# marvinli00/genie2

Hardware: AMD Instinct MI355X
Metric: denoise-steps/sec (N=256, T=1000, batch=8) (higher is better)
Workload: dtype f32 (pair-stack products as 3 f16 MFMAs on 2xf16-split operands, f32 accumulate); 1 GPU; unconditional N=256, T=1000, batch=8 per GPU, random-init base Denoiser (15.7M params), scale=0.6, reverse-loop steps 995..676; parallelism=replica per GPU x1, no data-path collective

## Files before the change

genie2_amd/csrc/common.h:

```cpp
#pragma once
#include <hip/hip_runtime.h>
#include <stdint.h>
#include "../../include/genie_hip.h"

typedef float f32x16 __attribute__((ext_vector_type(16)));
typedef float f32x4 __attribute__((ext_vector_type(4)));

#define GENIE_LN_EPS 1e-5f

#ifdef __HIPCC__

__device__ __forceinline__ f32x16 mfma_8k(const float4 a, const float4 b, f32x16 c) {
    c = __builtin_amdgcn_mfma_f32_32x32x2f32(a.x, b.x, c, 0, 0, 0);
    c = __builtin_amdgcn_mfma_f32_32x32x2f32(a.y, b.y, c, 0, 0, 0);
    c = __builtin_amdgcn_mfma_f32_32x32x2f32(a.z, b.z, c, 0, 0, 0);
    c = __builtin_amdgcn_mfma_f32_32x32x2f32(a.w, b.w, c, 0, 0, 0);
    return c;
}

__device__ __forceinline__ f32x16 zero16() {
    f32x16 z;
#pragma unroll
    for (int i = 0; i < 16; ++i) z[i] = 0.f;
    return z;
// ... 188 lines not shown
    int32_t *f_aatype, *f_rmask, *f_ridx, *f_cidx;
    float *f_pos;
    uint8_t *f_fsm, *f_fstm, *f_ifm;
    float *rmaskf;

    void* ws; size_t ws_bytes;
    float *p, *acm, *bcm, *xcm, *pstatic, *ipa_bias;
    float *spart;
    unsigned *pmax;
    float *xsingle, *s0, *s, *s1, *s2, *h1, *h2, *pij, *proj, *cat;
    float *kT, *v, *qp, *kpT, *vp;
    float *vf, *vmax;
    float *ta_tb, *ta_xn, *ta_qkvg;
    float *rots_w, *trans_w;
    int32_t* tsteps;
    float *loop_z;

    bool prof;
    struct ProfRec { int cls; hipEvent_t a, b; };
    ProfRec* prof_recs; int prof_n, prof_cap;
    double prof_ms[KC_COUNT]; int64_t prof_cnt[KC_COUNT];
    double train_gemm_flop;

    hipStream_t st2; hipEvent_t ev_fork, ev_join;
};

void launch_single_input(genie_ctx* h, hipStream_t st, const int32_t* timesteps);
void launch_gemm_rows(genie_ctx* h, hipStream_t st, const float* A, int lda, int M, int K,
                      const float* Wp, int Nout, const float* bias, const float* res, int ldr,
                      const float* rowmask, int relu, float* out, int ldo, int prof_class = KC_GEMM_ROWS);
// ... 4 lines not shown
                      const int8_t* codes);
void launch_trimul(genie_ctx* h, hipStream_t st, const TriMulW& w, bool outgoing);
void launch_pair_transition(genie_ctx* h, hipStream_t st, const PairLayerW& w);
void launch_triatt(genie_ctx* h, hipStream_t st, const TriAttW& w, bool starting);
void triatt_ws_floats(const genie_dims_t& d, int B, int N, size_t* tb, size_t* xn, size_t* qkvg);
bool launch_pair_stack_fused(genie_ctx* h, hipStream_t st, float* tap_trimul_out0, float* tap_layer0);
void launch_ipa_bias(genie_ctx* h, hipStream_t st);
void launch_ipa_prep(genie_ctx* h, hipStream_t st, int b0 = 0, int nb = -1);
void launch_ipa_attn(genie_ctx* h, hipStream_t st, int layer, const float* head_w, int b0 = 0, int nb = -1);
size_t ipa_vf_floats(const genie_dims_t& d, int B, int N);
bool ipa_attn_splits(const genie_ctx* h);
void launch_q_sample(genie_ctx* h, hipStream_t st, const float* x0, const float* z, const float* c0, const float* c1, float* trans_out);
void launch_training_loss(genie_ctx* h, hipStream_t st, const float* zp, const float* z, float w, float* losses, float* grad);
void launch_adam(hipStream_t st, size_t n, float* p, const float* g, float* m, float* v, double lr, double b1, double b2, double eps, int step);
void launch_any_nonzero(genie_ctx* h, hipStream_t st, const uint8_t* x, size_t n, unsigned* flag);
bool launch_struct_tail(genie_ctx* h, hipStream_t st, const StructLayerW& S, const float* trans_in, float* z_out, int b0 = 0, int nb = -1);
bool struct_tail_fused(const genie_ctx* h, const StructLayerW& S);
void launch_bb_update(genie_ctx* h, hipStream_t st, const StructLayerW& w, const float* trans_in,
                      float* z_out);
void launch_frenet(genie_ctx* h, hipStream_t st, int mode, int step, float scale, float* trans,
                   float* rots, const float* z, const float* eps);
void launch_fill_i32(genie_ctx* h, hipStream_t st, int32_t* p, int n, int v);
void train_ws_free(genie_ctx* h);

void prof_begin(genie_ctx* h, hipStream_t st, int cls);
void prof_end(genie_ctx* h, hipStream_t st);

struct ProfScope {
    genie_ctx* h; hipStream_t st; bool on;
    ProfScope(genie_ctx* h_, hipStream_t st_, int cls, bool enable = true) : h(h_), st(st_), on(enable && h_->prof) { if (on) prof_begin(h, st, cls); }
    ~ProfScope() { if (on) prof_end(h, st); }
};
```

genie2_amd/csrc/genie_api.hip:

```cpp
#include <stdio.h>
#include <stdlib.h>
#include <string.h>
#include <math.h>
#include <algorithm>
#include <cmath>
#include <new>
#include <string>
#include <vector>

#include "common.h"

void pair_kernels_init();
void pair_fused_kernels_init();
void single_kernels_init(const genie_dims_t& d, int n_max);
void launch_scale_copy(genie_ctx* h, hipStream_t st, const float* in, float* out, int n, float s);
size_t ipa_attn_lds(const genie_dims_t& d, int N);

static char g_create_err[512] = "";

#define SET_ERR(h, ...) do { snprintf((h)->err, sizeof((h)->err), __VA_ARGS__); } while (0)
#define HIP_TRY(h, call) do { hipError_t e_ = (call); if (e_ != hipSuccess) { \
    SET_ERR(h, "%s failed: %s (%s:%d)", #call, hipGetErrorString(e_), __FILE__, __LINE__); return GENIE_E_HIP; } } while (0)

static const char* kKernelNames[KC_COUNT] = {
// ... 96 lines not shown
}

static void free_batch(genie_ctx* h) {
    if (h->ws) { (void)hipFree(h->ws); h->ws = nullptr; h->ws_bytes = 0; }
    h->have_feats = false;
}

void genie_destroy(genie_handle_t h) {
    if (!h) return;
    (void)hipSetDevice(h->device);
    free_batch(h);
    train_ws_free(h);
    if (h->wdev) (void)hipFree(h->wdev);
    if (h->hxdev) (void)hipFree(h->hxdev);
    if (h->pos_tab) (void)hipFree(h->pos_tab);
    free(h->sched_host);
    for (int i = 0; i < h->prof_n; ++i) { (void)hipEventDestroy(h->prof_recs[i].a); (void)hipEventDestroy(h->prof_recs[i].b); }
    free(h->prof_recs);
    if (h->st2) { (void)hipStreamSynchronize(h->st2); (void)hipEventDestroy(h->ev_fork); (void)hipEventDestroy(h->ev_join); (void)hipStreamDestroy(h->st2); }
    delete[] h->pair;
    delete[] h->st;
    delete h;
}

const char* genie_last_error(genie_handle_t h) { return h ? h->err : g_create_err; }
size_t genie_workspace_bytes(genie_handle_t h) { return h ? h->ws_bytes : 0; }

namespace {
struct Img {
    std::vector<float> data;
// ... 380 lines not shown
    HIP_TRY(h, hipMemcpy(h->sched, sched, s * sizeof(float), hipMemcpyHostToDevice));
    free(h->sched_host);
    h->sched_host = (float*)malloc(s * sizeof(float));
    memcpy(h->sched_host, sched, s * sizeof(float));
    h->n_pos = n_pos;
    h->n_chain = n_chain;
    h->have_tables = true;
    return GENIE_OK;
}

__global__ void k_mask_to_float(const int32_t* m, float* f, int n) {
    const int i = blockIdx.x * blockDim.x + threadIdx.x;
    if (i < n) f[i] = (float)m[i];
}

int genie_prepare_features(genie_handle_t h, genie_stream_t stream, int B, int N, const genie_features_t* f) {
    if (!h || !f || B < 1 || N < 2) return GENIE_E_ARG;
    if (!h->have_weights) { SET_ERR(h, "genie_prepare_features: weights not loaded"); return GENIE_E_STATE; }
    const genie_dims_t& d = h->d;
    if (ipa_attn_lds(d, N) > 160 * 1024) { SET_ERR(h, "N = %d exceeds the attention kernel's LDS budget", N); return GENIE_E_ARG; }
    if ((size_t)24 * N * sizeof(float) > 160 * 1024) { SET_ERR(h, "N = %d exceeds the Frenet kernel's LDS budget (96 B per residue)", N); return GENIE_E_ARG; }
    {
        const size_t np = (size_t)((N + 31) / 32 * 32);
        const size_t pair_bytes = (size_t)B * np * np * d.c_p * sizeof(float);
        if (pair_bytes >= ((size_t)1 << 31)) {
            SET_ERR(h, "batch %d x N %d: a pair tensor of %zu bytes exceeds the 2 GiB the kernels address; split the batch", B, N, pair_bytes);
            return GENIE_E_ARG;
        }
    }
    HIP_TRY(h, hipSetDevice(h->device));
// ... 25 lines not shown
        size_t ntb, nxn, nq;
        triatt_ws_floats(d, B, N, &ntb, &nxn, &nq);
        want(&h->ta_tb, ntb * 4); want(&h->ta_xn, nxn * 4); want(&h->ta_qkvg, nq * 4);
    }
    size_t total = 0;
    for (auto& s : segs) total += s.bytes;
    if (total > h->ws_bytes) {
        free_batch(h);
        hipError_t e = hipMalloc(&h->ws, total);
        if (e != hipSuccess) { SET_ERR(h, "workspace hipMalloc(%zu MB) failed: %s", total >> 20, hipGetErrorString(e)); return GENIE_E_NOMEM; }
        h->ws_bytes = total;
    }
    size_t off = 0;
    for (auto& s : segs) { *s.p = (char*)h->ws + off; off += s.bytes; }
    h->B = B; h->N = N; h->NP = NP;

    HIP_TRY(h, hipMemcpyAsync(h->f_aatype, f->aatype, M * 20 * 4, hipMemcpyDeviceToDevice, st));
    HIP_TRY(h, hipMemcpyAsync(h->f_pos, f->atom_positions, M * 3 * 4, hipMemcpyDeviceToDevice, st));
    HIP_TRY(h, hipMemcpyAsync(h->f_rmask, f->residue_mask, M * 4, hipMemcpyDeviceToDevice, st));
    HIP_TRY(h, hipMemcpyAsync(h->f_ridx, f->residue_index, M * 4, hipMemcpyDeviceToDevice, st));
    HIP_TRY(h, hipMemcpyAsync(h->f_cidx, f->chain_index, M * 4, hipMemcpyDeviceToDevice, st));
    HIP_TRY(h, hipMemcpyAsync(h->f_fsm, f->fixed_sequence_mask, M, hipMemcpyDeviceToDevice, st));
    HIP_TRY(h, hipMemcpyAsync(h->f_fstm, f->fixed_structure_mask, P, hipMemcpyDeviceToDevice, st));
    HIP_TRY(h, hipMemcpyAsync(h->f_ifm, f->interface_mask, M, hipMemcpyDeviceToDevice, st));
    hipLaunchKernelGGL(k_mask_to_float, dim3((unsigned)((M + 255) / 256)), dim3(256), 0, st, h->f_rmask, h->rmaskf, (int)M);
    HIP_TRY(h, hipMemsetAsync(h->acm, 0, (size_t)B * cp * NP * NP * 4, st));
    HIP_TRY(h, hipMemsetAsync(h->vf, 0, ipa_vf_floats(d, B, N) * 4, st));
    HIP_TRY(h, hipMemsetAsync(h->bcm, 0, (size_t)B * cp * NP * NP * 4, st));
    single_kernels_init(d, N);
    {
        unsigned any = 0;
        HIP_TRY(h, hipMemsetAsync(h->pmax, 0, sizeof(unsigned), st));
        launch_any_nonzero(h, st, h->f_fstm, P, h->pmax);
        HIP_TRY(h, hipMemcpyAsync(&any, h->pmax, sizeof(unsigned), hipMemcpyDeviceToHost, st));
        HIP_TRY(h, hipStreamSynchronize(st));
        h->has_motif = any != 0;
    }
    launch_pair_static(h, st);
    HIP_TRY(h, hipGetLastError());
    h->have_feats = true;
    return GENIE_OK;
}

static int denoise_internal(genie_ctx* h, hipStream_t st, const float* trans, const float* rots, const int32_t* ts_dev,
                            const int8_t* codes, float* z_out, const genie_taps_t* taps) {
    const genie_dims_t& d = h->d;
    const int B = h->B, N = h->N, M = B * N;
    const size_t P = (size_t)M * N;
    const int cs = d.c_s, cp = d.c_p;
    const int ldx = (single_in(d) + 7) / 8 * 8;
    auto d2d = [&](void* dst, const void* src, size_t bytes) { return hipMemcpyAsync(dst, src, bytes, hipMemcpyDeviceToDevice, st); };

    h->hx_launches = 1;
    launch_scale_copy(h, st, trans, h->trans_w, M * 3, d.rescale);
    HIP_TRY(h, d2d(h->rots_w, rots, (size_t)M * 9 * 4));

    launch_single_input(h, st, ts_dev);
    launch_gemm_rows(h, st, h->xsingle, ldx, M, ldx, h->single_w, cs, nullptr, nullptr, 0, h->rmaskf, 0, h->s0, cs);
    if (taps && taps->s) HIP_TRY(h, d2d(taps->s, h->s0, (size_t)M * cs * 4));

    launch_gemm_rows(h, st, h->s0, cs, M, cs, h->pij_w, 2 * cp, nullptr, nullptr, 0, nullptr, 0, h->pij, 2 * cp);
    launch_pair_init(h, st, h->trans_w, h->rots_w, codes);
    if (taps && taps->p_init) HIP_TRY(h, d2d(taps->p_init, h->p, P * cp * 4));

    const bool fused = launch_pair_stack_fused(h, st, taps ? taps->p_trimul_out0 : nullptr, taps ? taps->p_layer0 : nullptr);
    for (int l = 0; l < (fused ? 0 : d.n_pair_transform_layer); ++l) {
        launch_trimul(h, st, h->pair[l].out, true);
        if (l == 0 && taps && taps->p_trimul_out0) HIP_TRY(h, d2d(taps->p_trimul_out0, h->p, P * cp * 4));
        launch_trimul(h, st, h->pair[l].in, false);
        if (d.n_head_tri > 0) {
            launch_triatt(h, st, h->pair[l].ta_start, true);
            launch_triatt(h, st, h->pair[l].ta_end, false);
            if (l == 0 && taps && taps->p_tri_att0) HIP_TRY(h, d2d(taps->p_tri_att0, h->p, P * cp * 4));
        }
        launch_pair_transition(h, st, h->pair[l]);
        if (l == 0 && taps && taps->p_layer0) HIP_TRY(h, d2d(taps->p_layer0, h->p, P * cp * 4));
    }
    if (taps && taps->p) HIP_TRY(h, d2d(taps->p, h->p, P * cp * 4));

    launch_ipa_bias(h, st);
    HIP_TRY(h, d2d(h->s, h->s0, (size_t)M * cs * 4));
    if (taps && taps->states) HIP_TRY(h, d2d(taps->states, h->s0, (size_t)M * cs * 4));
    int n_state = 1;
    const int nproj = ipa_proj_n(d), ncat = ipa_cat_n(d);
    bool split = h->st2 && B >= 2 && M >= 1024 && ipa_attn_splits(h) && !getenv("GENIE_NO_STRUCT_SPLIT");
    for (int l = 0; split && l < d.n_structure_layer; ++l) split = struct_tail_fused(h, h->st[l]);
    const int n_half = split ? 2 : 1;
    const int n_layers = d.n_structure_block * d.n_structure_layer;
    hipStream_t hstream[2] = {st, h->st2};
    if (split) {
        HIP_TRY(h, hipEventRecord(h->ev_fork, st));
        HIP_TRY(h, hipStreamWaitEvent(h->st2, h->ev_fork, 0));
    }
    for (int half = 0; half < n_half; ++half) {
        hipStream_t hs = hstream[half];
        const int b0 = (int)((long long)B * half / n_half), nb = (int)((long long)B * (half + 1) / n_half) - b0;
        const size_t r0 = (size_t)b0 * N, nr = (size_t)nb * N;
        int li = 0;
        for (int blk = 0; blk < d.n_structure_block; ++blk) {
            for (int l = 0; l < d.n_structure_layer; ++l, ++li) {
                const StructLayerW& S = h->st[l];
                const bool last = li == n_layers - 1;
                launch_gemm_rows(h, hs, h->s + r0 * cs, cs, (int)nr, cs, S.proj_w, nproj, S.proj_b, nullptr, 0, nullptr, 0, h->proj + r0 * nproj, nproj);
                launch_ipa_prep(h, hs, b0, nb);
                launch_ipa_attn(h, hs, l, S.head_w, b0, nb);
                if (li == 0 && taps && taps->ipa_cat0) HIP_TRY(h, hipMemcpyAsync(taps->ipa_cat0 + r0 * ncat, h->cat + r0 * ncat, nr * ncat * 4, hipMemcpyDeviceToDevice, hs));
                auto state_tap = [&]() -> hipError_t {
                    return (taps && taps->states) ? hipMemcpyAsync(taps->states + (size_t)(1 + li) * M * cs + r0 * cs, h->s + r0 * cs, nr * cs * 4, hipMemcpyDeviceToDevice, hs)
                                                  : hipSuccess;
                };
                if (launch_struct_tail(h, hs, S, last ? trans : nullptr, last ? z_out : nullptr, b0, nb)) { HIP_TRY(h, state_tap()); continue; }
                launch_gemm_rows(h, hs, h->cat, ncat, M, ncat, S.out_w, cs, S.out_b, h->s, cs, nullptr, 0, h->s1, cs);
                launch_layernorm_rows(h, hs, h->s1, h->s2, M, cs, S.ln_ipa_g, S.ln_ipa_b);
                launch_gemm_rows(h, hs, h->s2, cs, M, cs, S.t1_w, cs, S.t1_b, nullptr, 0, nullptr, 1, h->h1, cs);
                launch_gemm_rows(h, hs, h->h1, cs, M, cs, S.t2_w, cs, S.t2_b, nullptr, 0, nullptr, 1, h->h2, cs);
                launch_gemm_rows(h, hs, h->h2, cs, M, cs, S.t3_w, cs, S.t3_b, h->s2, cs, nullptr, 0, h->s1, cs);
                launch_layernorm_rows(h, hs, h->s1, h->s, M, cs, S.ln_tr_g, S.ln_tr_b);
                launch_bb_update(h, hs, S, last ? trans : nullptr, last ? z_out : nullptr);
                HIP_TRY(h, state_tap());
            }
        }
    }
    if (split) {
        for (int q = 1; q < n_half; ++q) {
            HIP_TRY(h, hipEventRecord(h->ev_join, hstream[q]));
            HIP_TRY(h, hipStreamWaitEvent(st, h->ev_join, 0));
// ... 75 lines not shown
                      int first_step, int last_step, float* trans_io, float* rots_io, float* record) {
    if (int rc = check_ready(h, "genie_sample_loop")) return rc;
    const int T = h->d.n_timestep;
    if (!noise || !trans_io || !rots_io || first_step > T || last_step < 1 || first_step < last_step) {
        SET_ERR(h, "genie_sample_loop: bad argument");
        return GENIE_E_ARG;
    }
    hipStream_t st = (hipStream_t)stream;
    const size_t n3 = (size_t)h->B * h->N * 3, nn = (size_t)h->B * h->N * h->N;
    if (first_step == T) {
        HIP_TRY(h, hipMemcpyAsync(trans_io, noise, n3 * 4, hipMemcpyDeviceToDevice, st));
        launch_frenet(h, st, 0, 0, 0.f, trans_io, rots_io, nullptr, nullptr);
    }
    int it = 0;
    for (int step = first_step; step >= last_step; --step, ++it) {
        launch_fill_i32(h, st, h->tsteps, h->B, step);
        const int8_t* codes = quat_codes ? quat_codes + (size_t)it * nn : nullptr;
        if (int rc = denoise_internal(h, st, trans_io, rots_io, h->tsteps, codes, h->loop_z, nullptr)) return rc;
        const float* eps = (step == 1) ? nullptr : noise + (size_t)(T - step + 1) * n3;
        launch_frenet(h, st, 1, step, scale, trans_io, rots_io, h->loop_z, eps);
        if (record) HIP_TRY(h, hipMemcpyAsync(record + (size_t)it * n3, trans_io, n3 * 4, hipMemcpyDeviceToDevice, st));
    }
    HIP_TRY(h, hipGetLastError());
    return GENIE_OK;
}

int genie_set_math(genie_handle_t h, int mode) {
    if (!h || (mode != GENIE_MATH_F32 && mode != GENIE_MATH_HX)) return GENIE_E_ARG;
    h->hx = mode == GENIE_MATH_HX;
    return GENIE_OK;
}
int genie_get_math(genie_handle_t h) { return h && h->hx ? GENIE_MATH_HX : GENIE_MATH_F32; }

int genie_profile_enable(genie_handle_t h, int enable) {
    if (!h) return GENIE_E_ARG;
// ... 27 lines not shown
```

genie2_amd/csrc/pair_hx_kernels.hip:

```cpp
#include "hx_pair.h"


template <int NW>
__global__ __launch_bounds__(NW * 64, NW == 8 ? 1 : 2) void k_pair_transition_hx(
    float* __restrict__ z, const float* __restrict__ rmask, const unsigned char* __restrict__ wimg,
    const float* __restrict__ b1s, const float* __restrict__ b2s, int N, long long M, int n_hb, float sx, float c1, float c2, int rev) {
    extern __shared__ __attribute__((aligned(16))) unsigned char smb[];
    float* sb1 = reinterpret_cast<float*>(smb + 2 * HX_STAGE_BYTES);
    const int lane = threadIdx.x & 63, wave = UNI(threadIdx.x >> 6);
    const int h = lane >> 5, pl = lane & 31;
    const int n_wt = (int)((M + 31) / 32);
    const int n_tiles = (n_wt + NW - 1) / NW;
    const rsrc_t rw = hx_rsrc(wimg, (unsigned)(n_hb * HX_STAGE_BYTES));
    const rsrc_t rz = hx_rsrc(z, (unsigned)(M * 512));
    const rsrc_t rnull = hx_rsrc(z, 0u);
    const int lane16 = lane * 16;
    constexpr int PW = 32 / NW;
    auto issue = [&](int hb, int buf) {
#pragma unroll
        for (int q = 0; q < PW; ++q) {
            const int p = PW * wave + q;
            hx_dma(rw, smb + buf * HX_STAGE_BYTES + p * 1024, lane16, hb * HX_STAGE_BYTES + p * 1024);
        }
    };
// ... 807 lines not shown
    }
#pragma unroll
    for (int o = 32; o > 0; o >>= 1) amax = fmaxf(amax, __shfl_xor(amax, o));
    if (lane == 0 && __float_as_uint(amax) > *reinterpret_cast<volatile unsigned*>(pmax)) atomicMax(pmax, __float_as_uint(amax));
}

bool launch_ipa_bias_hx(genie_ctx* h, hipStream_t st) {
    const int LH = h->d.n_structure_layer * h->d.n_head_ipa;
    if (!h->hx || LH > 96) return false;
    const HxGemmW* w = nullptr;
    for (int i = 0; i < h->n_hxg; ++i)
        if (h->hxg[i].w == h->ipa_bias_w) w = &h->hxg[i];
    if (!w) return false;
    const int N = h->N, n_tiles = h->B * N * ((N + 31) / 32);
    const int grid = n_tiles / 4 < 2 * hx_num_cu() ? (n_tiles + 3) / 4 : 2 * hx_num_cu();
    (void)hipMemsetAsync(h->pmax, 0, sizeof(unsigned), st);
    hipLaunchKernelGGL(k_ipa_bias_hx, dim3(grid), dim3(256), IB_UNITS * 2048 + 96 * 4, st, h->p, w->img, w->inv_s, h->ipa_bias_b, h->ipa_bias,
                       h->B, N, LH, n_tiles, (int)(h->hx_launches & 1), h->pmax);
    return true;
}

void pair_hx_kernels_init() {
#define HX_ATTR(k) (void)hipFuncSetAttribute(reinterpret_cast<const void*>(k), hipFuncAttributeMaxDynamicSharedMemorySize, HX_LDS_BYTES)
    HX_ATTR((k_trimul_proj_hx<true, 8>)); HX_ATTR((k_trimul_proj_hx<false, 8>));
    HX_ATTR(k_trimul_out_hx_r<8>);
    (void)hipFuncSetAttribute(reinterpret_cast<const void*>(k_trimul_contract_hx_big), hipFuncAttributeMaxDynamicSharedMemorySize, 4 * CB_PLANE);
#undef HX_ATTR
    (void)hipFuncSetAttribute(reinterpret_cast<const void*>(k_pair_transition_hx<8>), hipFuncAttributeMaxDynamicSharedMemorySize, HX_LDS_BYTES);
    (void)hipFuncSetAttribute(reinterpret_cast<const void*>(k_ipa_bias_hx), hipFuncAttributeMaxDynamicSharedMemorySize, IB_UNITS * 2048 + 96 * 4);
}
```

genie2_amd/csrc/pair_kernels.hip:

```cpp
#include "common.h"

#define LDZ 132


template <bool AMAX = false>
__device__ __forceinline__ float load_tile64(float* tile, const float* __restrict__ src, size_t row_stride,
                                             int nvalid, int tid) {
    const int c4 = tid & 31;
    const int r0 = tid >> 5;
    float4 v[8];
    const int last = max(nvalid - 1, 0);
#pragma unroll
    for (int u = 0; u < 8; ++u) {
        const int r = min(r0 + 8 * u, last);
        v[u] = *reinterpret_cast<const float4*>(src + (size_t)r * row_stride + c4 * 4);
    }
#pragma unroll
    for (int u = 0; u < 8; ++u) {
        const int r = r0 + 8 * u;
        if (r >= nvalid) v[u] = make_float4(0.f, 0.f, 0.f, 0.f);
        *reinterpret_cast<float4*>(tile + r * LDZ + c4 * 4) = v[u];
    }
    float am = 0.f;
    if constexpr (AMAX) {
// ... 181 lines not shown
#pragma unroll
    for (int q = 0; q < 10; ++q) {
        const int k = part + 4 * q;
        if (k < nbin) frow[k] = (x[q] / s) * pm;
    }
}

#define LDF 52
template <bool TABLE>
__global__ __launch_bounds__(256) void k_pair_init(const float* __restrict__ trans, const float* __restrict__ rots,
                                                   const int8_t* __restrict__ codes, const float* __restrict__ rmask,
                                                   const uint8_t* __restrict__ fstm, const float* __restrict__ pij,
                                                   const float* __restrict__ pstatic, const float* __restrict__ wt,
                                                   float* __restrict__ p, int N, float dmin, float dstep, int nbin,
                                                   const int32_t* __restrict__ ridx, const int32_t* __restrict__ cidx,
                                                   const float* __restrict__ relpos_t, int relpos_k) {
    __shared__ __attribute__((aligned(16))) float ft[64 * LDF];
    __shared__ float pmk[64];
    __shared__ int dsel[64];
    __shared__ float same[64];
    const int tid = threadIdx.x, lane = tid & 63, wave = tid >> 6;
    const int ntile = (N + 63) >> 6;
    const int st = blockIdx.x % ntile;
    const int i = (blockIdx.x / ntile) % N;
    const int b = blockIdx.x / (ntile * N);
    const int t0 = st * 64;
    const int nvalid = min(64, N - t0);
    {
        const int jl = tid >> 2, part = tid & 3;
        float* frow = ft + jl * LDF;
        if (jl < nvalid) {
            const int j = t0 + jl;
            const float pm = rmask[b * N + i] * rmask[b * N + j];
            const float* xi = trans + ((size_t)b * N + i) * 3;
            const float* xj = trans + ((size_t)b * N + j) * 3;
            const float dx = xi[0] - xj[0], dy = xi[1] - xj[1], dz = xi[2] - xj[2];
            const float d = sqrtf(1e-10f + ((dx * dx + dy * dy) + dz * dz));
            soft_bins(frow, d, dmin, dstep, nbin, pm, part);
            if (part == 0) {
                const float* Ri = rots + ((size_t)b * N + i) * 9;
                const float* Rj = rots + ((size_t)b * N + j) * 9;
                float r[9];
// ... 139 lines not shown
        hipLaunchKernelGGL(k_pair_static<true>, grid, dim3(256), 0, st, h->f_pos, h->f_ridx, h->f_cidx, h->f_fsm, h->f_fstm,
                           h->relpos_t, h->motif_w, h->pstatic, N, h->d.relpos_k, h->d.template_dist_min,
                           h->d.template_dist_step, h->d.template_dist_n_bin);
    else
        hipLaunchKernelGGL(k_pair_static<false>, grid, dim3(256), 0, st, h->f_pos, h->f_ridx, h->f_cidx, h->f_fsm, h->f_fstm,
                           h->relpos_t, h->motif_w, h->pstatic, N, h->d.relpos_k, h->d.template_dist_min,
                           h->d.template_dist_step, h->d.template_dist_n_bin);
}

void launch_pair_init(genie_ctx* h, hipStream_t st, const float* trans, const float* rots, const int8_t* codes) {
    ProfScope ps(h, st, KC_PAIR_INIT);
    const int N = h->N, ntile = (N + 63) / 64;
    if (!h->has_motif)
        hipLaunchKernelGGL(k_pair_init<true>, dim3(h->B * N * ntile), dim3(256), 0, st, trans, rots, codes, h->rmaskf, h->f_fstm,
                           h->pij, h->pstatic, h->templ_w, h->p, N, h->d.template_dist_min, h->d.template_dist_step,
                           h->d.template_dist_n_bin, h->f_ridx, h->f_cidx, h->relpos_t, h->d.relpos_k);
    else
        hipLaunchKernelGGL(k_pair_init<false>, dim3(h->B * N * ntile), dim3(256), 0, st, trans, rots, codes, h->rmaskf, h->f_fstm,
                           h->pij, h->pstatic, h->templ_w, h->p, N, h->d.template_dist_min, h->d.template_dist_step,
                           h->d.template_dist_n_bin, h->f_ridx, h->f_cidx, h->relpos_t, h->d.relpos_k);
}

void launch_trimul_proj_wl(genie_ctx* h, hipStream_t st, const TriMulW& w, bool outgoing);
void launch_trimul_out_wl(genie_ctx* h, hipStream_t st, const TriMulW& w);
void launch_pair_transition_wl(genie_ctx* h, hipStream_t st, const PairLayerW& w);

void launch_trimul_hx(genie_ctx* h, hipStream_t st, const TriMulW& w, bool outgoing);
void launch_trimul(genie_ctx* h, hipStream_t st, const TriMulW& w, bool outgoing) {
    if (h->hx) { launch_trimul_hx(h, st, w, outgoing); return; }
    const int NP = h->NP;
    {
        ProfScope ps(h, st, KC_TRIMUL_PROJ);
        launch_trimul_proj_wl(h, st, w, outgoing);
    }
    {
// ... 24 lines not shown

void launch_pair_transition_hx(genie_ctx* h, hipStream_t st, const PairLayerW& w);
void launch_pair_transition(genie_ctx* h, hipStream_t st, const PairLayerW& w) {
    ProfScope ps(h, st, KC_PAIR_TRANSITION);
    if (h->hx) launch_pair_transition_hx(h, st, w);
    else launch_pair_transition_wl(h, st, w);
}

bool launch_ipa_bias_hx(genie_ctx* h, hipStream_t st);
void launch_ipa_bias(genie_ctx* h, hipStream_t st) {
    ProfScope ps(h, st, KC_IPA_BIAS);
    if (launch_ipa_bias_hx(h, st)) return;
    const int N = h->N, ntile = (N + 127) / 128;
    const int LH = h->d.n_structure_layer * h->d.n_head_ipa;
    const size_t lds = 128 * LDZ * sizeof(float);
    (void)hipMemsetAsync(h->pmax, 0, sizeof(unsigned), st);
    hipLaunchKernelGGL(k_ipa_bias, dim3(h->B * N * ntile), dim3(256), lds, st, h->p, h->ipa_bias_w, h->ipa_bias_b, h->ipa_bias,
                       h->B, N, LH, h->hx ? (int)(h->hx_launches & 1) : 0, h->pmax);
}

void pair_wl_kernels_init();
void pair_hx_kernels_init();
void pair_kernels_init() {
    pair_wl_kernels_init();
    pair_hx_kernels_init();
    (void)hipFuncSetAttribute(reinterpret_cast<const void*>(k_trimul_contract<2>), hipFuncAttributeMaxDynamicSharedMemorySize,
                        2 * 2 * 128 * LDK * sizeof(float));
    (void)hipFuncSetAttribute(reinterpret_cast<const void*>(k_ipa_bias), hipFuncAttributeMaxDynamicSharedMemorySize,
                        128 * LDZ * sizeof(float));
}
```

genie2_amd/csrc/single_kernels.hip:

```cpp
#include <algorithm>
#include <type_traits>
#include "hx.h"

__global__ void k_single_input(float* __restrict__ x, int ldx, const float* __restrict__ pos_tab, int n_pos, int c_pos,
                               const float* __restrict__ chain_tab, int n_chain, int c_chain,
                               const float* __restrict__ t_tab, int c_t, const int32_t* __restrict__ timesteps,
                               const int32_t* __restrict__ ridx, const int32_t* __restrict__ cidx,
                               const int32_t* __restrict__ aatype, const uint8_t* __restrict__ fsm,
                               const uint8_t* __restrict__ ifm, int N, int n_timestep) {
    const int row = blockIdx.x;
    const int b = row / N;
    float* xr = x + (size_t)row * ldx;
    const int ri = min(max(ridx[row], 0), n_pos - 1);
    const int ci = min(max(cidx[row], 0), n_chain - 1);
    const int ts = min(max(timesteps[b], 0), n_timestep);
    const float f = fsm[row] ? 1.f : 0.f;
    const int o1 = c_pos, o2 = o1 + c_chain, o3 = o2 + c_t, o4 = o3 + 20;
    for (int c = threadIdx.x; c < ldx; c += blockDim.x) {
        float v;
        if (c < o1) v = pos_tab[(size_t)ri * c_pos + c];
        else if (c < o2) v = chain_tab[(size_t)ci * c_chain + (c - o1)];
        else if (c < o3) v = t_tab[(size_t)ts * c_t + (c - o2)];
        else if (c < o4) v = (float)aatype[(size_t)row * 20 + (c - o3)] * f;
        else if (c < o4 + 2) v = f;
// ... 961 lines not shown
            for (int k = 0; k < 9; ++k) R[k] = Rn[k];
            t[0] = tx; t[1] = ty; t[2] = tz;
            if (z_out) {
                z_out[(size_t)row * 3 + 0] = trans_in[(size_t)row * 3 + 0] - tx * inv_rescale;
                z_out[(size_t)row * 3 + 1] = trans_in[(size_t)row * 3 + 1] - ty * inv_rescale;
                z_out[(size_t)row * 3 + 2] = trans_in[(size_t)row * 3 + 2] - tz * inv_rescale;
            }
        }
    }
}

__global__ __launch_bounds__(256) void k_p_sample_frenet(int mode, float* __restrict__ trans, float* __restrict__ rots,
                                                         const float* __restrict__ z, const float* __restrict__ eps,
                                                         const int32_t* __restrict__ rmask, const int32_t* __restrict__ cidx,
                                                         int N, float alpha, float sqrt_alpha, float somac, float sqrt_beta,
                                                         float scale) {
    extern __shared__ __attribute__((aligned(16))) float sm[];
    float* x = sm;
    float* tv = x + 3 * N;
    float* base = tv + 3 * N;
    float* st1 = base + 9 * N;
    __shared__ int s_len;
    const int b = blockIdx.x, tid = threadIdx.x;
    float* tr = trans + (size_t)b * N * 3;
    if (tid == 0) s_len = 0;
    __syncthreads();
    int cnt = 0;
    for (int n = tid; n < N; n += 256) cnt += rmask[b * N + n];
    atomicAdd(&s_len, cnt);
    if (mode == 1) {
        const float w_z = (1.0f - alpha) / somac;
        const float inv_sa = 1.0f / sqrt_alpha;
        for (int u = tid; u < 3 * N; u += 256) {
            const float m = (float)rmask[b * N + u / 3];
            float v = inv_sa * (tr[u] - w_z * z[(size_t)b * N * 3 + u]);
            v = v * m;
            if (eps) { v = v + scale * sqrt_beta * eps[(size_t)b * N * 3 + u]; v = v * m; }
            x[u] = v;
            tr[u] = v;
        }
    } else {
        for (int u = tid; u < 3 * N; u += 256) x[u] = tr[u];
    }
    __syncthreads();
    const int len = s_len;
    for (int n = tid; n < N - 1; n += 256) {
        const float dx = x[3 * n + 3] - x[3 * n], dy = x[3 * n + 4] - x[3 * n + 1], dz = x[3 * n + 5] - x[3 * n + 2];
        const float nr = sqrtf(1e-10f + ((dx * dx + dy * dy) + dz * dz));
        tv[3 * n] = dx / nr; tv[3 * n + 1] = dy / nr; tv[3 * n + 2] = dz / nr;
    }
    __syncthreads();
    for (int n = tid; n < N; n += 256) {
        float R[9] = {1.f, 0.f, 0.f, 0.f, 1.f, 0.f, 0.f, 0.f, 1.f};
        if (n >= 1 && n < len - 1) {
            const int m = n - 1;
            const float ax = tv[3 * m], ay = tv[3 * m + 1], az = tv[3 * m + 2];
            const float bx = tv[3 * m + 3], by = tv[3 * m + 4], bz = tv[3 * m + 5];
            float cx = ay * bz - az * by, cy = az * bx - ax * bz, cz = ax * by - ay * bx;
// ... 13 lines not shown
        int srcn = n;
        if (n < len && (n == 0 || ch[n] != ch[n - 1])) srcn = n + 1;
#pragma unroll
        for (int k = 0; k < 9; ++k) st1[9 * n + k] = (srcn < N) ? base[9 * srcn + k] : ((k % 4 == 0) ? 1.f : 0.f);
    }
    __syncthreads();
    float* ro = rots + (size_t)b * N * 9;
    for (int n = tid; n < N; n += 256) {
        int k = n;
        if (n < len) {
            while (k >= 0 && (k == len - 1 || ch[k] != ch[k + 1])) --k;
            if (k < 0) k = N - 1;
        }
#pragma unroll
        for (int q = 0; q < 9; ++q) ro[9 * n + q] = st1[9 * k + q];
    }
}

__global__ void k_fill_i32(int32_t* p, int n, int v) {
    const int i = blockIdx.x * blockDim.x + threadIdx.x;
    if (i < n) p[i] = v;
}

__global__ void k_scale_copy(const float* __restrict__ in, float* __restrict__ out, int n, float s) {
    const int i = blockIdx.x * blockDim.x + threadIdx.x;
    if (i < n) out[i] = in[i] * s;
}

template <int H, int C, int PQ, int PV, int Q, int MF>
__global__ __launch_bounds__(MF ? 128 * Q : 512, MF ? 4 : 1) void k_ipa_attn_q(const float* __restrict__ proj, int ldp, const float* __restrict__ kT,
                                                    const float* __restrict__ v, const float* __restrict__ qp,
                                                    const float* __restrict__ kpT, const float* __restrict__ vp,
                                                    const float* __restrict__ bias, const float* __restrict__ z,
                                                    const float* __restrict__ rots, const float* __restrict__ trans,
                                                    const float* __restrict__ rmask, const float* __restrict__ head_w,
                                                    float* __restrict__ cat, int B, int N, int layer, int rev,
// ... 550 lines not shown
    const int M = h->B * h->N;
    hipLaunchKernelGGL(k_bb_update, dim3((M + 3) / 4), dim3(256), 0, st, h->s, h->d.c_s, w.bb_w, w.bb_b, h->rots_w, h->trans_w,
                       M, trans_in, z_out, 1.0f / h->d.rescale);
}

static size_t struct_rows_lds() { return (size_t)2 * 32 * SR_LD * 4 + 6 * (2 * 32 * GH_ROWB + 32 * 4) + 32 * 12 * 4; }
static const HxGemmW* hx_image(const genie_ctx* h, const float* Wp) {
    for (int i = 0; i < h->n_hxg; ++i)
        if (h->hxg[i].w == Wp) return &h->hxg[i];
    return nullptr;
}
bool struct_tail_fused(const genie_ctx* h, const StructLayerW& S) {
    if (!h->hx || h->d.c_s != 384 || getenv("GENIE_NO_STRUCT_FUSE")) return false;
    return hx_image(h, S.out_w) && hx_image(h, S.t1_w) && hx_image(h, S.t2_w) && hx_image(h, S.t3_w);
}
bool launch_struct_tail(genie_ctx* h, hipStream_t st, const StructLayerW& S, const float* trans_in, float* z_out, int b0, int nb) {
    if (!struct_tail_fused(h, S)) return false;
    const HxGemmW *w0 = hx_image(h, S.out_w), *w1 = hx_image(h, S.t1_w), *w2 = hx_image(h, S.t2_w), *w3 = hx_image(h, S.t3_w);
    if (nb < 0) { b0 = 0; nb = h->B; }
    const int Mall = h->B * h->N, M = nb * h->N, cs = h->d.c_s, ncat = h->d.n_head_ipa * (h->d.c_p + h->d.c_hidden_ipa + 4 * h->d.n_v_point);
    const size_t zs = (size_t)Mall * cs, r0 = (size_t)b0 * h->N;
    {
        ProfScope ps(h, st, KC_GEMM_ROWS);
        hipLaunchKernelGGL(k_gemm_rows_hx, dim3((M + 31) / 32, (cs + 127) / 128, SR_KSPLIT), dim3(256), 0, st, h->cat + r0 * ncat, ncat, M, ncat,
                           w0->img, cs, w0->inv_s, nullptr, nullptr, 0, nullptr, 0, h->spart + r0 * cs, cs, zs);
    }
    ProfScope ps(h, st, KC_STRUCT_ROWS);
    const int nrb = (M + 31) / 32;
    hipLaunchKernelGGL((k_struct_rows_hx<12>), dim3(nrb + 64), dim3(768), struct_rows_lds(), st, h->spart + r0 * cs, SR_KSPLIT, zs, S.out_b, h->s + r0 * cs,
                       S.ln_ipa_g, S.ln_ipa_b, w1->img, w1->inv_s, S.t1_b, w2->img, w2->inv_s, S.t2_b, w3->img, w3->inv_s, S.t3_b,
                       S.ln_tr_g, S.ln_tr_b, S.bb_w, S.bb_b, h->s + r0 * cs, h->rots_w + r0 * 9, h->trans_w + r0 * 3, M, trans_in ? trans_in + r0 * 3 : nullptr,
                       z_out ? z_out + r0 * 3 : nullptr, 1.0f / h->d.rescale, nrb);
    return true;
}

void launch_q_sample(genie_ctx* h, hipStream_t st, const float* x0, const float* z, const float* c0, const float* c1, float* trans_out) {
    ProfScope ps(h, st, KC_MISC);
    const int total = h->B * h->N * 3;
    hipLaunchKernelGGL(k_q_sample, dim3((total + 255) / 256), dim3(256), 0, st, x0, z, c0, c1, trans_out, h->N * 3, total);
}
void launch_training_loss(genie_ctx* h, hipStream_t st, const float* zp, const float* z, float w, float* losses, float* grad) {
    ProfScope ps(h, st, KC_MISC);
    float* stats = h->loop_z;
    hipLaunchKernelGGL(k_training_loss, dim3(h->B), dim3(256), 0, st, zp, z, h->f_rmask, h->f_fsm, h->B, h->N, w, losses, stats, grad);
    hipLaunchKernelGGL(k_training_loss_mean, dim3(1), dim3(64), 0, st, stats, h->B, losses);
}

void launch_frenet(genie_ctx* h, hipStream_t st, int mode, int step, float scale, float* trans, float* rots, const float* z,
                   const float* eps) {
    ProfScope ps(h, st, KC_P_SAMPLE);
    float al = 1.f, sa = 1.f, so = 1.f, sb = 0.f;
    if (mode == 1) {
        const int T1 = h->d.n_timestep + 1;
        al = h->sched_host[0 * T1 + step];
        sa = h->sched_host[1 * T1 + step];
        so = h->sched_host[2 * T1 + step];
        sb = h->sched_host[3 * T1 + step];
    }
    const size_t lds = (size_t)(3 + 3 + 9 + 9) * h->N * sizeof(float);
    hipLaunchKernelGGL(k_p_sample_frenet, dim3(h->B), dim3(256), lds, st, mode, trans, rots, z, eps, h->f_rmask, h->f_cidx, h->N,
                       al, sa, so, sb, scale);
}

int genie_frenet_frames(genie_stream_t stream, int B, int N, const float* coords, const int32_t* chains, const int32_t* mask,
                        float* rots_out) {
    if (!coords || !chains || !mask || !rots_out || B < 1 || N < 2) return GENIE_E_ARG;
    const size_t lds = (size_t)24 * N * sizeof(float);
    if (lds > 160 * 1024) return GENIE_E_ARG;
    if (lds > 64 * 1024)
        (void)hipFuncSetAttribute(reinterpret_cast<const void*>(k_p_sample_frenet), hipFuncAttributeMaxDynamicSharedMemorySize, (int)lds);
    hipLaunchKernelGGL(k_p_sample_frenet, dim3(B), dim3(256), lds, (hipStream_t)stream, 0, const_cast<float*>(coords), rots_out,
                       (const float*)nullptr, (const float*)nullptr, mask, chains, N, 1.f, 1.f, 1.f, 0.f, 0.f);
    return hipGetLastError() == hipSuccess ? GENIE_OK : GENIE_E_HIP;
}

void launch_fill_i32(genie_ctx* h, hipStream_t st, int32_t* p, int n, int v) {
    ProfScope ps(h, st, KC_MISC);
    hipLaunchKernelGGL(k_fill_i32, dim3((n + 255) / 256), dim3(256), 0, st, p, n, v);
}

void launch_scale_copy(genie_ctx* h, hipStream_t st, const float* in, float* out, int n, float s) {
    ProfScope ps(h, st, KC_MISC);
    hipLaunchKernelGGL(k_scale_copy, dim3((n + 255) / 256), dim3(256), 0, st, in, out, n, s);
}

void single_kernels_init(const genie_dims_t& d, int n_max) {
    (void)hipFuncSetAttribute(reinterpret_cast<const void*>(k_p_sample_frenet), hipFuncAttributeMaxDynamicSharedMemorySize,
                        (int)std::min<size_t>((size_t)24 * n_max * sizeof(float), 160 * 1024));
    (void)hipFuncSetAttribute(reinterpret_cast<const void*>(k_struct_rows_hx<12>), hipFuncAttributeMaxDynamicSharedMemorySize,
                        (int)struct_rows_lds());
    if (ipa_is_base(d)) {
        if (ipa_use_q(d, n_max)) {
            (void)hipFuncSetAttribute(reinterpret_cast<const void*>(k_ipa_attn_q<12, 16, 4, 8, IPA_Q, 0>),
// ... 11 lines not shown
```

Measured before the change: 113.0 batch-steps/s.

## Remove per-step small launches and copies from the denoise loop

Removes several tiny per-step operations from the reverse sampling loop. A precomputed device timestep table replaces the per-step fill kernel. The frenet sampling kernel now writes the rescaled trans and rots working copies for the next step, so the scale-copy and the rots memcpy are skipped after the first step. The pmax memset is folded into the pair-init kernel, and the s0-to-s copy is dropped when the fused struct tail can read s0 directly. This cuts launch and dispatch overhead, but it couples the frenet and struct kernels to buffer state that carries across steps.

```diff
diff --git a/genie2_amd/csrc/common.h b/genie2_amd/csrc/common.h
--- a/genie2_amd/csrc/common.h
+++ b/genie2_amd/csrc/common.h
@@ -226,6 +226,7 @@
     float *ta_tb, *ta_xn, *ta_qkvg;
     float *rots_w, *trans_w;
     int32_t* tsteps;
+    int32_t* ts_tab; size_t ts_tab_n;
     float *loop_z;
 
     bool prof;
@@ -260,13 +261,13 @@
 void launch_training_loss(genie_ctx* h, hipStream_t st, const float* zp, const float* z, float w, float* losses, float* grad);
 void launch_adam(hipStream_t st, size_t n, float* p, const float* g, float* m, float* v, double lr, double b1, double b2, double eps, int step);
 void launch_any_nonzero(genie_ctx* h, hipStream_t st, const uint8_t* x, size_t n, unsigned* flag);
-bool launch_struct_tail(genie_ctx* h, hipStream_t st, const StructLayerW& S, const float* trans_in, float* z_out, int b0 = 0, int nb = -1);
+bool launch_struct_tail(genie_ctx* h, hipStream_t st, const StructLayerW& S, const float* trans_in, float* z_out, int b0 = 0, int nb = -1,
+                        const float* s_in = nullptr);
 bool struct_tail_fused(const genie_ctx* h, const StructLayerW& S);
 void launch_bb_update(genie_ctx* h, hipStream_t st, const StructLayerW& w, const float* trans_in,
                       float* z_out);
 void launch_frenet(genie_ctx* h, hipStream_t st, int mode, int step, float scale, float* trans,
-                   float* rots, const float* z, const float* eps);
-void launch_fill_i32(genie_ctx* h, hipStream_t st, int32_t* p, int n, int v);
+                   float* rots, const float* z, const float* eps, float* trans_w = nullptr, float* rots_w = nullptr);
 void train_ws_free(genie_ctx* h);
 
 void prof_begin(genie_ctx* h, hipStream_t st, int cls);
diff --git a/genie2_amd/csrc/genie_api.hip b/genie2_amd/csrc/genie_api.hip
--- a/genie2_amd/csrc/genie_api.hip
+++ b/genie2_amd/csrc/genie_api.hip
@@ -134,6 +134,7 @@
     if (h->wdev) (void)hipFree(h->wdev);
     if (h->hxdev) (void)hipFree(h->hxdev);
     if (h->pos_tab) (void)hipFree(h->pos_tab);
+    if (h->ts_tab) (void)hipFree(h->ts_tab);
     free(h->sched_host);
     for (int i = 0; i < h->prof_n; ++i) { (void)hipEventDestroy(h->prof_recs[i].a); (void)hipEventDestroy(h->prof_recs[i].b); }
     free(h->prof_recs);
@@ -544,6 +545,11 @@
     if (i < n) f[i] = (float)m[i];
 }
 
+__global__ void k_timestep_table(int32_t* tab, int n, int B) {
+    const int i = blockIdx.x * blockDim.x + threadIdx.x;
+    if (i < n) tab[i] = i / B;
+}
+
 int genie_prepare_features(genie_handle_t h, genie_stream_t stream, int B, int N, const genie_features_t* f) {
     if (!h || !f || B < 1 || N < 2) return GENIE_E_ARG;
     if (!h->have_weights) { SET_ERR(h, "genie_prepare_features: weights not loaded"); return GENIE_E_STATE; }
@@ -599,6 +605,15 @@
     size_t off = 0;
     for (auto& s : segs) { *s.p = (char*)h->ws + off; off += s.bytes; }
     h->B = B; h->N = N; h->NP = NP;
+    {
+        const size_t nts = (size_t)(d.n_timestep + 1) * B;
+        if (nts > h->ts_tab_n) {
+            if (h->ts_tab) (void)hipFree(h->ts_tab);
+            h->ts_tab = nullptr; h->ts_tab_n = 0;
+            if (hipMalloc(&h->ts_tab, nts * 4) != hipSuccess) { SET_ERR(h, "timestep table hipMalloc(%zu B) failed", nts * 4); return GENIE_E_NOMEM; }
+            h->ts_tab_n = nts;
+        }
+    }
 
     HIP_TRY(h, hipMemcpyAsync(h->f_aatype, f->aatype, M * 20 * 4, hipMemcpyDeviceToDevice, st));
     HIP_TRY(h, hipMemcpyAsync(h->f_pos, f->atom_positions, M * 3 * 4, hipMemcpyDeviceToDevice, st));
@@ -609,6 +624,8 @@
     HIP_TRY(h, hipMemcpyAsync(h->f_fstm, f->fixed_structure_mask, P, hipMemcpyDeviceToDevice, st));
     HIP_TRY(h, hipMemcpyAsync(h->f_ifm, f->interface_mask, M, hipMemcpyDeviceToDevice, st));
     hipLaunchKernelGGL(k_mask_to_float, dim3((unsigned)((M + 255) / 256)), dim3(256), 0, st, h->f_rmask, h->rmaskf, (int)M);
+    hipLaunchKernelGGL(k_timestep_table, dim3((unsigned)(((size_t)(d.n_timestep + 1) * B + 255) / 256)), dim3(256), 0, st, h->ts_tab,
+                       (d.n_timestep + 1) * B, B);
     HIP_TRY(h, hipMemsetAsync(h->acm, 0, (size_t)B * cp * NP * NP * 4, st));
     HIP_TRY(h, hipMemsetAsync(h->vf, 0, ipa_vf_floats(d, B, N) * 4, st));
     HIP_TRY(h, hipMemsetAsync(h->bcm, 0, (size_t)B * cp * NP * NP * 4, st));
@@ -628,7 +645,7 @@
 }
 
 static int denoise_internal(genie_ctx* h, hipStream_t st, const float* trans, const float* rots, const int32_t* ts_dev,
-                            const int8_t* codes, float* z_out, const genie_taps_t* taps) {
+                            const int8_t* codes, float* z_out, const genie_taps_t* taps, bool frames_ready = false) {
     const genie_dims_t& d = h->d;
     const int B = h->B, N = h->N, M = B * N;
     const size_t P = (size_t)M * N;
@@ -637,8 +654,10 @@
     auto d2d = [&](void* dst, const void* src, size_t bytes) { return hipMemcpyAsync(dst, src, bytes, hipMemcpyDeviceToDevice, st); };
 
     h->hx_launches = 1;
-    launch_scale_copy(h, st, trans, h->trans_w, M * 3, d.rescale);
-    HIP_TRY(h, d2d(h->rots_w, rots, (size_t)M * 9 * 4));
+    if (!frames_ready) {
+        launch_scale_copy(h, st, trans, h->trans_w, M * 3, d.rescale);
+        HIP_TRY(h, d2d(h->rots_w, rots, (size_t)M * 9 * 4));
+    }
 
     launch_single_input(h, st, ts_dev);
     launch_gemm_rows(h, st, h->xsingle, ldx, M, ldx, h->single_w, cs, nullptr, nullptr, 0, h->rmaskf, 0, h->s0, cs);
@@ -664,12 +683,13 @@
     if (taps && taps->p) HIP_TRY(h, d2d(taps->p, h->p, P * cp * 4));
 
     launch_ipa_bias(h, st);
-    HIP_TRY(h, d2d(h->s, h->s0, (size_t)M * cs * 4));
     if (taps && taps->states) HIP_TRY(h, d2d(taps->states, h->s0, (size_t)M * cs * 4));
     int n_state = 1;
     const int nproj = ipa_proj_n(d), ncat = ipa_cat_n(d);
     bool split = h->st2 && B >= 2 && M >= 1024 && ipa_attn_splits(h) && !getenv("GENIE_NO_STRUCT_SPLIT");
     for (int l = 0; split && l < d.n_structure_layer; ++l) split = struct_tail_fused(h, h->st[l]);
+    const bool s0_direct = struct_tail_fused(h, h->st[0]);
+    if (!s0_direct) HIP_TRY(h, d2d(h->s, h->s0, (size_t)M * cs * 4));
     const int n_half = split ? 2 : 1;
     const int n_layers = d.n_structure_block * d.n_structure_layer;
     hipStream_t hstream[2] = {st, h->st2};
@@ -686,7 +706,8 @@
             for (int l = 0; l < d.n_structure_layer; ++l, ++li) {
                 const StructLayerW& S = h->st[l];
                 const bool last = li == n_layers - 1;
-                launch_gemm_rows(h, hs, h->s + r0 * cs, cs, (int)nr, cs, S.proj_w, nproj, S.proj_b, nullptr, 0, nullptr, 0, h->proj + r0 * nproj, nproj);
+                const float* s_in = (li == 0 && s0_direct) ? h->s0 : h->s;
+                launch_gemm_rows(h, hs, s_in + r0 * cs, cs, (int)nr, cs, S.proj_w, nproj, S.proj_b, nullptr, 0, nullptr, 0, h->proj + r0 * nproj, nproj);
                 launch_ipa_prep(h, hs, b0, nb);
                 launch_ipa_attn(h, hs, l, S.head_w, b0, nb);
                 if (li == 0 && taps && taps->ipa_cat0) HIP_TRY(h, hipMemcpyAsync(taps->ipa_cat0 + r0 * ncat, h->cat + r0 * ncat, nr * ncat * 4, hipMemcpyDeviceToDevice, hs));
@@ -694,7 +715,7 @@
                     return (taps && taps->states) ? hipMemcpyAsync(taps->states + (size_t)(1 + li) * M * cs + r0 * cs, h->s + r0 * cs, nr * cs * 4, hipMemcpyDeviceToDevice, hs)
                                                   : hipSuccess;
                 };
-                if (launch_struct_tail(h, hs, S, last ? trans : nullptr, last ? z_out : nullptr, b0, nb)) { HIP_TRY(h, state_tap()); continue; }
+                if (launch_struct_tail(h, hs, S, last ? trans : nullptr, last ? z_out : nullptr, b0, nb, s_in)) { HIP_TRY(h, state_tap()); continue; }
                 launch_gemm_rows(h, hs, h->cat, ncat, M, ncat, S.out_w, cs, S.out_b, h->s, cs, nullptr, 0, h->s1, cs);
                 launch_layernorm_rows(h, hs, h->s1, h->s2, M, cs, S.ln_ipa_g, S.ln_ipa_b);
                 launch_gemm_rows(h, hs, h->s2, cs, M, cs, S.t1_w, cs, S.t1_b, nullptr, 0, nullptr, 1, h->h1, cs);
@@ -800,11 +821,11 @@
     }
     int it = 0;
     for (int step = first_step; step >= last_step; --step, ++it) {
-        launch_fill_i32(h, st, h->tsteps, h->B, step);
         const int8_t* codes = quat_codes ? quat_codes + (size_t)it * nn : nullptr;
-        if (int rc = denoise_internal(h, st, trans_io, rots_io, h->tsteps, codes, h->loop_z, nullptr)) return rc;
+        if (int rc = denoise_internal(h, st, trans_io, rots_io, h->ts_tab + (size_t)step * h->B, codes, h->loop_z, nullptr, it > 0)) return rc;
         const float* eps = (step == 1) ? nullptr : noise + (size_t)(T - step + 1) * n3;
-        launch_frenet(h, st, 1, step, scale, trans_io, rots_io, h->loop_z, eps);
+        const bool more = step > last_step;
+        launch_frenet(h, st, 1, step, scale, trans_io, rots_io, h->loop_z, eps, more ? h->trans_w : nullptr, more ? h->rots_w : nullptr);
         if (record) HIP_TRY(h, hipMemcpyAsync(record + (size_t)it * n3, trans_io, n3 * 4, hipMemcpyDeviceToDevice, st));
     }
     HIP_TRY(h, hipGetLastError());
diff --git a/genie2_amd/csrc/pair_hx_kernels.hip b/genie2_amd/csrc/pair_hx_kernels.hip
--- a/genie2_amd/csrc/pair_hx_kernels.hip
+++ b/genie2_amd/csrc/pair_hx_kernels.hip
@@ -845,7 +845,6 @@
     if (!w) return false;
     const int N = h->N, n_tiles = h->B * N * ((N + 31) / 32);
     const int grid = n_tiles / 4 < 2 * hx_num_cu() ? (n_tiles + 3) / 4 : 2 * hx_num_cu();
-    (void)hipMemsetAsync(h->pmax, 0, sizeof(unsigned), st);
     hipLaunchKernelGGL(k_ipa_bias_hx, dim3(grid), dim3(256), IB_UNITS * 2048 + 96 * 4, st, h->p, w->img, w->inv_s, h->ipa_bias_b, h->ipa_bias,
                        h->B, N, LH, n_tiles, (int)(h->hx_launches & 1), h->pmax);
     return true;
diff --git a/genie2_amd/csrc/pair_kernels.hip b/genie2_amd/csrc/pair_kernels.hip
--- a/genie2_amd/csrc/pair_kernels.hip
+++ b/genie2_amd/csrc/pair_kernels.hip
@@ -219,7 +219,7 @@
                                                    const float* __restrict__ pstatic, const float* __restrict__ wt,
                                                    float* __restrict__ p, int N, float dmin, float dstep, int nbin,
                                                    const int32_t* __restrict__ ridx, const int32_t* __restrict__ cidx,
-                                                   const float* __restrict__ relpos_t, int relpos_k) {
+                                                   const float* __restrict__ relpos_t, int relpos_k, unsigned* __restrict__ pmax) {
     __shared__ __attribute__((aligned(16))) float ft[64 * LDF];
     __shared__ float pmk[64];
     __shared__ int dsel[64];
@@ -231,6 +231,7 @@
     const int b = blockIdx.x / (ntile * N);
     const int t0 = st * 64;
     const int nvalid = min(64, N - t0);
+    if (blockIdx.x == 0 && tid == 0) *pmax = 0u;
     {
         const int jl = tid >> 2, part = tid & 3;
         float* frow = ft + jl * LDF;
@@ -400,11 +401,11 @@
     if (!h->has_motif)
         hipLaunchKernelGGL(k_pair_init<true>, dim3(h->B * N * ntile), dim3(256), 0, st, trans, rots, codes, h->rmaskf, h->f_fstm,
                            h->pij, h->pstatic, h->templ_w, h->p, N, h->d.template_dist_min, h->d.template_dist_step,
-                           h->d.template_dist_n_bin, h->f_ridx, h->f_cidx, h->relpos_t, h->d.relpos_k);
+                           h->d.template_dist_n_bin, h->f_ridx, h->f_cidx, h->relpos_t, h->d.relpos_k, h->pmax);
     else
         hipLaunchKernelGGL(k_pair_init<false>, dim3(h->B * N * ntile), dim3(256), 0, st, trans, rots, codes, h->rmaskf, h->f_fstm,
                            h->pij, h->pstatic, h->templ_w, h->p, N, h->d.template_dist_min, h->d.template_dist_step,
-                           h->d.template_dist_n_bin, h->f_ridx, h->f_cidx, h->relpos_t, h->d.relpos_k);
+                           h->d.template_dist_n_bin, h->f_ridx, h->f_cidx, h->relpos_t, h->d.relpos_k, h->pmax);
 }
 
 void launch_trimul_proj_wl(genie_ctx* h, hipStream_t st, const TriMulW& w, bool outgoing);
@@ -459,7 +460,6 @@
     const int N = h->N, ntile = (N + 127) / 128;
     const int LH = h->d.n_structure_layer * h->d.n_head_ipa;
     const size_t lds = 128 * LDZ * sizeof(float);
-    (void)hipMemsetAsync(h->pmax, 0, sizeof(unsigned), st);
     hipLaunchKernelGGL(k_ipa_bias, dim3(h->B * N * ntile), dim3(256), lds, st, h->p, h->ipa_bias_w, h->ipa_bias_b, h->ipa_bias,
                        h->B, N, LH, h->hx ? (int)(h->hx_launches & 1) : 0, h->pmax);
 }
diff --git a/genie2_amd/csrc/single_kernels.hip b/genie2_amd/csrc/single_kernels.hip
--- a/genie2_amd/csrc/single_kernels.hip
+++ b/genie2_amd/csrc/single_kernels.hip
@@ -999,7 +999,7 @@
                                                          const float* __restrict__ z, const float* __restrict__ eps,
                                                          const int32_t* __restrict__ rmask, const int32_t* __restrict__ cidx,
                                                          int N, float alpha, float sqrt_alpha, float somac, float sqrt_beta,
-                                                         float scale) {
+                                                         float scale, float* __restrict__ trans_w, float* __restrict__ rots_w, float rescale) {
     extern __shared__ __attribute__((aligned(16))) float sm[];
     float* x = sm;
     float* tv = x + 3 * N;
@@ -1027,6 +1027,9 @@
     } else {
         for (int u = tid; u < 3 * N; u += 256) x[u] = tr[u];
     }
+    if (trans_w) {
+        for (int u = tid; u < 3 * N; u += 256) trans_w[(size_t)b * N * 3 + u] = x[u] * rescale;
+    }
     __syncthreads();
     const int len = s_len;
     for (int n = tid; n < N - 1; n += 256) {
@@ -1070,12 +1073,11 @@
         }
 #pragma unroll
         for (int q = 0; q < 9; ++q) ro[9 * n + q] = st1[9 * k + q];
-    }
-}
-
-__global__ void k_fill_i32(int32_t* p, int n, int v) {
-    const int i = blockIdx.x * blockDim.x + threadIdx.x;
-    if (i < n) p[i] = v;
+        if (rots_w) {
+#pragma unroll
+            for (int q = 0; q < 9; ++q) rots_w[((size_t)b * N + n) * 9 + q] = st1[9 * k + q];
+        }
+    }
 }
 
 __global__ void k_scale_copy(const float* __restrict__ in, float* __restrict__ out, int n, float s) {
@@ -1656,7 +1658,7 @@
     if (!h->hx || h->d.c_s != 384 || getenv("GENIE_NO_STRUCT_FUSE")) return false;
     return hx_image(h, S.out_w) && hx_image(h, S.t1_w) && hx_image(h, S.t2_w) && hx_image(h, S.t3_w);
 }
-bool launch_struct_tail(genie_ctx* h, hipStream_t st, const StructLayerW& S, const float* trans_in, float* z_out, int b0, int nb) {
+bool launch_struct_tail(genie_ctx* h, hipStream_t st, const StructLayerW& S, const float* trans_in, float* z_out, int b0, int nb, const float* s_in) {
     if (!struct_tail_fused(h, S)) return false;
     const HxGemmW *w0 = hx_image(h, S.out_w), *w1 = hx_image(h, S.t1_w), *w2 = hx_image(h, S.t2_w), *w3 = hx_image(h, S.t3_w);
     if (nb < 0) { b0 = 0; nb = h->B; }
@@ -1669,7 +1671,7 @@
     }
     ProfScope ps(h, st, KC_STRUCT_ROWS);
     const int nrb = (M + 31) / 32;
-    hipLaunchKernelGGL((k_struct_rows_hx<12>), dim3(nrb + 64), dim3(768), struct_rows_lds(), st, h->spart + r0 * cs, SR_KSPLIT, zs, S.out_b, h->s + r0 * cs,
+    hipLaunchKernelGGL((k_struct_rows_hx<12>), dim3(nrb + 64), dim3(768), struct_rows_lds(), st, h->spart + r0 * cs, SR_KSPLIT, zs, S.out_b, (s_in ? s_in : h->s) + r0 * cs,
                        S.ln_ipa_g, S.ln_ipa_b, w1->img, w1->inv_s, S.t1_b, w2->img, w2->inv_s, S.t2_b, w3->img, w3->inv_s, S.t3_b,
                        S.ln_tr_g, S.ln_tr_b, S.bb_w, S.bb_b, h->s + r0 * cs, h->rots_w + r0 * 9, h->trans_w + r0 * 3, M, trans_in ? trans_in + r0 * 3 : nullptr,
                        z_out ? z_out + r0 * 3 : nullptr, 1.0f / h->d.rescale, nrb);
@@ -1689,7 +1691,7 @@
 }
 
 void launch_frenet(genie_ctx* h, hipStream_t st, int mode, int step, float scale, float* trans, float* rots, const float* z,
-                   const float* eps) {
+                   const float* eps, float* trans_w, float* rots_w) {
     ProfScope ps(h, st, KC_P_SAMPLE);
     float al = 1.f, sa = 1.f, so = 1.f, sb = 0.f;
     if (mode == 1) {
@@ -1701,7 +1703,7 @@
     }
     const size_t lds = (size_t)(3 + 3 + 9 + 9) * h->N * sizeof(float);
     hipLaunchKernelGGL(k_p_sample_frenet, dim3(h->B), dim3(256), lds, st, mode, trans, rots, z, eps, h->f_rmask, h->f_cidx, h->N,
-                       al, sa, so, sb, scale);
+                       al, sa, so, sb, scale, trans_w, rots_w, h->d.rescale);
 }
 
 int genie_frenet_frames(genie_stream_t stream, int B, int N, const float* coords, const int32_t* chains, const int32_t* mask,
@@ -1712,13 +1714,8 @@
     if (lds > 64 * 1024)
         (void)hipFuncSetAttribute(reinterpret_cast<const void*>(k_p_sample_frenet), hipFuncAttributeMaxDynamicSharedMemorySize, (int)lds);
     hipLaunchKernelGGL(k_p_sample_frenet, dim3(B), dim3(256), lds, (hipStream_t)stream, 0, const_cast<float*>(coords), rots_out,
-                       (const float*)nullptr, (const float*)nullptr, mask, chains, N, 1.f, 1.f, 1.f, 0.f, 0.f);
+                       (const float*)nullptr, (const float*)nullptr, mask, chains, N, 1.f, 1.f, 1.f, 0.f, 0.f, (float*)nullptr, (float*)nullptr, 1.f);
     return hipGetLastError() == hipSuccess ? GENIE_OK : GENIE_E_HIP;
-}
-
-void launch_fill_i32(genie_ctx* h, hipStream_t st, int32_t* p, int n, int v) {
-    ProfScope ps(h, st, KC_MISC);
-    hipLaunchKernelGGL(k_fill_i32, dim3((n + 255) / 256), dim3(256), 0, st, p, n, v);
 }
 
 void launch_scale_copy(genie_ctx* h, hipStream_t st, const float* in, float* out, int n, float s) {
```

New measurement: 113.2 batch-steps/s (median of 6 runs). About the same (+0.2%).
